# VITA-Group/LightGaussian

Hardware: AMD Instinct MI355X
Metric: views/sec fwd+bwd @1080p (N Gaussians) (higher is better)
Workload: dtype f32; 1 GPU; 3000000 synthetic Gaussians (SURVEY 8d generator, seed 20250103), 1920x1080, SH degree 3, fwdbwd through gaussian_renderer.render, 200-camera orbit; n_gaussians=3000000, width=1920, height=1080, mode=fwdbwd, views=200, exp=hardware, loss=L1 (HIP, lg_loss_forward/backward with LG_FLAG_L1_ONLY), parallelism=camera-shard x1

## Files before the change

### include/lightgaussian.h

```cpp
#ifndef LIGHTGAUSSIAN_H
#define LIGHTGAUSSIAN_H

#include <stddef.h>
#include <stdint.h>

#ifdef __cplusplus
extern "C" {
#endif

#define LG_ABI_VERSION 7

enum {
    LG_OK = 0,
    LG_ERR_INVALID_ARGUMENT = -1,
    LG_ERR_DEVICE = -2,
    LG_ERR_ALLOC = -3,
    LG_ERR_PREFILTERED = -4
};

enum { LG_WEIGHT_ONE = 0, LG_WEIGHT_OPACITY = 1, LG_WEIGHT_ALPHA = 2, LG_WEIGHT_ALPHA_T = 3 };

enum {
    LG_FLAG_DEBUG = 1,
    LG_FLAG_FAST_EXP = 2,
    LG_FLAG_PROFILE = 4,
    LG_FLAG_SKIP_COLOR = 16,
    LG_FLAG_L1_ONLY = 32,
    LG_FLAG_NARROW_KEY = 64,
    LG_FLAG_SORT_ALL_BITS = 128,
    LG_FLAG_K1_LDS = 256,
    LG_FLAG_LONG_SERIAL = 512,
    LG_FLAG_LONG_PARALLEL = 1024,
    LG_FLAG_SAVE_SH_JACOBIAN = 2048,
    LG_FLAG_COUNT_WIDE_BAND = 8192,
    LG_FLAG_RAW_PARAMS = 8
};

typedef struct lg_view {
    int32_t image_height;
    int32_t image_width;
    float tanfovx;
    float tanfovy;
    const float* bg;
    float scale_modifier;
    const float* viewmatrix;
    const float* projmatrix;
    int32_t sh_degree;
    const float* campos;
    int32_t prefiltered;
// ... 116 lines not shown
```

### lightgaussian_amd/_lib.py

```python
import ctypes as C
import os
import subprocess

_HERE = os.path.dirname(os.path.abspath(__file__))
LIB_PATH = os.environ.get("LIGHTGAUSSIAN_HIP_LIB") or os.path.join(_HERE, "liblightgaussian_hip.so")

LG_OK = 0
LG_ERR_INVALID_ARGUMENT = -1
LG_ERR_DEVICE = -2
LG_ERR_ALLOC = -3
LG_ERR_PREFILTERED = -4

WEIGHT_ONE, WEIGHT_OPACITY, WEIGHT_ALPHA, WEIGHT_ALPHA_T = 0, 1, 2, 3
FLAG_DEBUG, FLAG_FAST_EXP, FLAG_PROFILE, FLAG_RAW_PARAMS, FLAG_SKIP_COLOR, FLAG_L1_ONLY = 1, 2, 4, 8, 16, 32
FLAG_NARROW_KEY, FLAG_SORT_ALL_BITS, FLAG_K1_LDS = 64, 128, 256
FLAG_LONG_SERIAL, FLAG_LONG_PARALLEL = 512, 1024
FLAG_SAVE_SH_JACOBIAN = 2048
FLAG_COUNT_WIDE_BAND = 8192
ABI_VERSION = 7

EXPORTS = ["lg_geom_bytes", "lg_img_bytes", "lg_binning_bytes", "lg_backward_scratch_bytes", "lg_forward",
           "lg_forward_count", "lg_backward", "lg_score_from_count", "lg_abi_version", "lg_last_error",
           "lg_profile_read", "lg_profile_reset", "lg_last_stats", "lg_debug_reduce9", "lg_loss_state_bytes",
           "lg_loss_forward", "lg_loss_backward", "lg_prune_scratch_bytes", "lg_prune_epilogue", "lg_knn_scratch_bytes",
           "lg_knn3_mean_dist2", "lg_ordered_sum", "lg_forward_bounded", "lg_select_mask", "lg_compact_scratch_bytes",
           "lg_compact_plan", "lg_compact_rows", "lg_vq_scratch_bytes", "lg_vq_nearest", "lg_debug_sort_temp_bytes",
           "lg_debug_sort_keys", "lg_build_id", "lg_backward_chunked", "lg_debug_activations", "lg_view_status",
           "lg_debug_sort_orphan", "lg_debug_last_contributor", "lg_debug_tile_lists", "lg_geom_visible_offset",
           "lg_sh_grad_from_rgb", "lg_debug_view_meta", "lg_vq_ema_scratch_bytes", "lg_vq_ema_step", "lg_vq_colors"]


class lg_view(C.Structure):
    _fields_ = [("image_height", C.c_int32), ("image_width", C.c_int32), ("tanfovx", C.c_float), ("tanfovy", C.c_float),
# ... 146 lines not shown
```

### lightgaussian_amd/csrc/lg_api.hip

```cpp
#include "lg_host.h"
#include "lg_wave.h"
#include "lg_preprocess.h"
#include "lg_binning.h"
#include "lg_blend.h"
#include "lg_loss.h"
#include "lg_prune.h"
#include "lg_knn.h"
#include "lg_compact.h"
#include "lg_vq.h"
#include "lg_vq_train.h"
#include "lg_vq_color.h"

struct ViewGeom { int W, H, gx, gy, ntiles, ntiles_pad, S, gid_bits; uint32_t gid_mask; };
static ViewGeom view_geom(const lg_view* v, int N)
{
    ViewGeom q;
    q.W = v->image_width; q.H = v->image_height;
    q.gx = (q.W + LG_TILE - 1) / LG_TILE; q.gy = (q.H + LG_TILE - 1) / LG_TILE;
    q.ntiles = (int)((int64_t)q.gx * q.gy);
    q.ntiles_pad = (int)(((int64_t)q.ntiles + LG_TILE_GRID_ALIGN - 1) / LG_TILE_GRID_ALIGN * LG_TILE_GRID_ALIGN);
    q.S = lg_segment_of(v);
    q.gid_bits = lg_gid_bits(N);
    q.gid_mask = lg_gid_mask(q.gid_bits);
    return q;
// ... 44 lines not shown
            if (!g_pin_free.empty()) { p = g_pin_free.back().first; ev = g_pin_free.back().second; g_pin_free.pop_back(); }
        }
        if (!p) {
            if (hipHostMalloc((void**)&p, 64, hipHostMallocDefault) != hipSuccess) { p = nullptr; return; }
            if (hipEventCreateWithFlags(&ev, hipEventDisableTiming) != hipSuccess) { (void)hipHostFree(p); p = nullptr; ev = nullptr; }
        }
    }
    ~PinnedSlot()
    {
        if (p) { std::lock_guard<std::mutex> lk(g_pin_mu); g_pin_free.emplace_back(p, ev); }
    }
    PinnedSlot(const PinnedSlot&) = delete;
    PinnedSlot& operator=(const PinnedSlot&) = delete;
};

#define KCHECK(name)                                                                         \
    do {                                                                                     \
        hipError_t _e = hipGetLastError();                                                   \
        if (_e != hipSuccess) return fail(LG_ERR_DEVICE, name " launch", _e);                \
        if (debug) {                                                                         \
            _e = hipStreamSynchronize(stream);                                               \
            if (_e != hipSuccess) return fail(LG_ERR_DEVICE, name " execution", _e);         \
        }                                                                                    \
    } while (0)

#define LG_STATUS_PENDING 0xFFFFFFFFu

static_assert(LG_W_ALPHA == LG_WEIGHT_ALPHA && LG_W_ALPHA_T == LG_WEIGHT_ALPHA_T, "ForwardPlan::fscore is the kernels' FSCORE");
using PreprocessKernel = decltype(&lg_preprocess<false, false>);
static PreprocessKernel preprocess_kernel(bool raw, bool direct)
{
    static const PreprocessKernel k[2][2] = { { lg_preprocess<false, false>, lg_preprocess<false, true> }, { lg_preprocess<true, false>, lg_preprocess<true, true> } };
    return k[raw][direct];
}
using BlendFwdKernel = decltype(&lg_blend_fwd<false, 0, true, true>);
static BlendFwdKernel blend_fwd_kernel(const ForwardPlan& p)
{
    static const BlendFwdKernel color[2] = { lg_blend_fwd<false, 0, false, true>, lg_blend_fwd<false, 0, true, true> };
    static const BlendFwdKernel count_image[3][2] = { { lg_blend_fwd<true, 0, false, true>, lg_blend_fwd<true, 0, true, true> },
                                                      { lg_blend_fwd<true, LG_W_ALPHA, false, true>, lg_blend_fwd<true, LG_W_ALPHA, true, true> },
                                                      { lg_blend_fwd<true, LG_W_ALPHA_T, false, true>, lg_blend_fwd<true, LG_W_ALPHA_T, true, true> } };
    static const BlendFwdKernel significance[3] = { lg_blend_fwd<true, 0, true, false>, lg_blend_fwd<true, LG_W_ALPHA, true, false>,
                                                    lg_blend_fwd<true, LG_W_ALPHA_T, true, false> };
    const int w = p.fscore == LG_W_ALPHA ? 1 : p.fscore == LG_W_ALPHA_T ? 2 : 0;
    return !p.count ? color[p.exact] : p.color ? count_image[w][p.exact] : significance[w];
}
using BlendBwdKernel = decltype(&lg_blend_bwd<true>);
// ... 3 lines not shown
{
    static const PreprocessBwdKernel k[2][2] = { { lg_preprocess_bwd<false, false>, lg_preprocess_bwd<false, true> },
                                                 { lg_preprocess_bwd<true, false>, lg_preprocess_bwd<true, true> } };
    return k[raw][jac];
}

struct Bounded { void* binning; int64_t capacity; float max_depth; uint32_t* status; uint32_t* host_status; };

struct Forward {
    const lg_view* v; const lg_gaussians* g; const Bounded* bounded; lg_alloc_fn alloc; void* alloc_user; int weight_policy;
    float* out_color; int32_t* out_radii; int32_t* out_count; float* out_score; void** binning_out; int64_t* num_rendered;
    hipStream_t stream; bool debug, prof;
    int N, nblk; ViewGeom q; GeomView geo; ImgView img; BinView bin;
    KeyPlan kp; ForwardPlan plan;
    int64_t cap;
    bool k1_cleared_sort;
    PinnedSlot vslot;
    uint32_t* device_status() const { return bounded ? bounded->status : nullptr; }
    int front_end();
    int binning();
    int blend();
    int score();
    int epilogue();
};

int Forward::front_end()
{
    const bool count = out_count != nullptr;
    if (bounded) {
        if (!bounded->binning || bounded->capacity <= 0 || bounded->capacity >= (1ll << 30) || !(bounded->max_depth > 0.2f))
            return fail(LG_ERR_INVALID_ARGUMENT, "lg_forward_bounded: binning buffer, 0 < max_rendered < 2^30 and max_depth > 0.2 required");
        kp = make_key_plan(q.ntiles, N, __builtin_bit_cast(uint32_t, bounded->max_depth), v->flags);
        cap = bounded->capacity;
        bin = carve_bin(bounded->binning, cap, q.W, q.H, q.S);
        if (N == 0) {
            HIP_TRY(lg_zero_async(geo.counters, 16, stream));
            if (bounded->status) HIP_TRY(lg_zero_async(bounded->status, 16, stream));
            HIP_TRY(lg_zero_async(bin.ranges, (size_t)q.ntiles * 8, stream));
        }
    }
    plan = make_forward_plan(v->flags, count, weight_policy, N, bounded ? cap : 1);
    const bool host_words = bounded && bounded->host_status;
    if (host_words) {
        if (!vslot.p) return fail(LG_ERR_ALLOC, "hipHostMalloc of the status slot failed");
        if (N > 0) { vslot.p[1] = vslot.p[2] = vslot.p[3] = 0u; __atomic_store_n(&vslot.p[0], LG_STATUS_PENDING, __ATOMIC_RELEASE); }
        else memset(vslot.p, 0, 16);
    }
    uint32_t* k1_clear = nullptr;
    uint32_t k1_nclear = 0;
    if (bounded && plan.live) {
        k1_clear = (uint32_t*)bin.sort_temp;
        k1_nclear = (uint32_t)(lg_sort_clear_bytes(lg_sort_layout((size_t)cap), (unsigned)kp.sort_passes()) / 4);
    }
    k1_cleared_sort = k1_clear != nullptr;
    if (N > 0) {
        {
            ProfScope ps(prof, "preprocess", stream);
            const bool direct = !(v->flags & LG_FLAG_K1_LDS), raw = v->flags & LG_FLAG_RAW_PARAMS;
            const size_t k1_dyn = (direct && g->shs && !g->colors_precomp && !plan.k1_skip_color) ? LG_K1_PAD_LDS : 0;
            preprocess_kernel(raw, direct)<<<nblk, LG_PP, k1_dyn, stream>>>(
                N, g->M, v->sh_degree, q.W, q.H, v->tanfovx, v->tanfovy, v->scale_modifier, v->prefiltered, plan.k1_skip_color ? 1 : 0, v->viewmatrix,
                v->projmatrix, v->campos, g->means3D, g->shs, g->shs_rest, g->colors_precomp, g->opacities, g->scales, g->rotations, g->cov3D_precomp, geo,
                out_radii, plan.k1_clears_count ? out_count : nullptr, out_score, k1_clear, k1_nclear, (v->flags & LG_FLAG_SAVE_SH_JACOBIAN) ? 1 : 0);
        }
        KCHECK("lg_preprocess");
        {
            ProfScope ps(prof, "scan", stream);
            lg_scan_blocks<<<(nblk + LG_PART - 1) / LG_PART, LG_PART, 0, stream>>>(nblk, geo.blk_sum, geo.blk_dmax, geo.blk_off, geo.part_sum,
                                                                                  geo.part_dmax, geo.part_prefix, geo.counters + 8,
                                                                                  bounded ? (uint32_t)cap : 0xFFFFFFFFu,
                                                                                  bounded ? kp.depth_bits : 32, geo.counters,
                                                                                  host_words ? vslot.p : device_status());
        }
        KCHECK("lg_scan_blocks");
    }
    if (!bounded) {
        uint32_t h_counters[4] = {0, 0, 0, 0};
        if (N > 0) {
            PinnedSlot slot;
            if (!slot.p) return fail(LG_ERR_ALLOC, "hipHostMalloc of the read-back slot failed");
            HIP_TRY(hipMemcpyAsync(slot.p, geo.counters, 16, hipMemcpyDeviceToHost, stream));
            HIP_TRY(hipStreamSynchronize(stream));
            for (int k = 0; k < 4; k++) h_counters[k] = slot.p[k];
            if (v->prefiltered && h_counters[1]) return fail(LG_ERR_PREFILTERED, "Point is filtered although prefiltered is set. This shouldn't happen!");
            if (h_counters[0] & 1u) return fail(LG_ERR_INVALID_ARGUMENT, "more than 2^32-1 tile instances in one view");
        }
        cap = h_counters[3];
        if (cap >= (1ll << 30)) return fail(LG_ERR_INVALID_ARGUMENT, "more than 2^30-1 tile instances in one view");
        kp = make_key_plan(q.ntiles, N, h_counters[2], v->flags);
        plan = make_forward_plan(v->flags, count, weight_policy, N, cap);
        void* bin_p = alloc(alloc_user, carve_bin(nullptr, cap, q.W, q.H, q.S).total);
        if (!bin_p) return fail(LG_ERR_ALLOC, "binning allocator returned NULL");
        if (binning_out) *binning_out = bin_p;
        bin = carve_bin(bin_p, cap, q.W, q.H, q.S);
        if (num_rendered) *num_rendered = cap;
        if (cap == 0) HIP_TRY(lg_zero_async(bin.ranges, (size_t)q.ntiles * 8, stream));
    }
    g_stats.num_rendered = bounded ? -1 : cap;
    g_stats.num_visible = -1;
    return LG_OK;
}

int Forward::binning()
{
    if (!plan.live) return LG_OK;
    const int sort_begin = kp.sort_begin(), sort_end = kp.sort_end();
    const LgSortLayout SL = lg_sort_layout((size_t)cap);
    if (!k1_cleared_sort) HIP_TRY(lg_zero_async(bin.sort_temp, lg_sort_clear_bytes(SL, (unsigned)kp.sort_passes()), stream));
    uint32_t* hist = (uint32_t*)((char*)bin.sort_temp + SL.hist_off);
    {
        ProfScope ps(prof, "duplicate", stream);
        const int dgrid = std::max(1, std::min((nblk + 4 * LG_DUP_WAVES - 1) / (4 * LG_DUP_WAVES), LG_DUP_GRID));
        lg_duplicate<<<dgrid, LG_DUP_THREADS, 0, stream>>>(N, nblk, q.gx, kp.stored(), kp.store_drop, kp.gid_bits, sort_begin, sort_end, (uint32_t)cap, geo.touched,
                                                          geo.blk_off, geo.part_prefix, geo.counters, geo.offsets, geo.tinfo, bin.keys_in, q.ntiles, bin.ranges, hist,
// ... 109 lines not shown
    if (count && !out_score) return fail(LG_ERR_INVALID_ARGUMENT, "count needs score");
    if (count && (weight_policy < 0 || weight_policy > 3)) return fail(LG_ERR_INVALID_ARGUMENT, "bad weight policy");
    if (count && weight_policy >= LG_WEIGHT_ALPHA && (int64_t)v->image_width * v->image_height > (1ll << 24))
        return fail(LG_ERR_INVALID_ARGUMENT, "ALPHA / ALPHA_T weights: images beyond 2^24 pixels overflow the Q24.40 per-view sums");
    Forward f{};
    f.v = v; f.g = g; f.bounded = bounded; f.alloc = alloc; f.alloc_user = alloc_user; f.weight_policy = weight_policy;
    f.out_color = out_color; f.out_radii = out_radii; f.out_count = out_count; f.out_score = out_score;
    f.binning_out = binning_out; f.num_rendered = num_rendered;
    f.stream = (hipStream_t)stream_p; f.debug = v->flags & LG_FLAG_DEBUG; f.prof = v->flags & LG_FLAG_PROFILE;
    f.N = g->N; f.nblk = (f.N + LG_PP - 1) / LG_PP;
    f.q = view_geom(v, f.N);
    f.geo = carve_geom(geom_p, f.N);
    f.img = carve_img(img_p, f.q.W, f.q.H);
    if (binning_out) *binning_out = nullptr;
    if (num_rendered) *num_rendered = 0;
    if ((rc = f.front_end()) != LG_OK || (rc = f.binning()) != LG_OK || (rc = f.blend()) != LG_OK || (rc = f.score()) != LG_OK) return rc;
    return f.epilogue();
}


extern "C" int lg_forward(const lg_view* view, const lg_gaussians* g, void* geom, void* img, lg_alloc_fn alloc, void* alloc_user,
                          float* out_color, int32_t* out_radii, void** binning_out, int64_t* num_rendered, void* stream)
{
    return forward_impl(view, g, geom, img, alloc, alloc_user, nullptr, LG_WEIGHT_OPACITY, out_color, out_radii, nullptr, nullptr, binning_out,
                        num_rendered, stream);
}

extern "C" int lg_forward_count(const lg_view* view, const lg_gaussians* g, void* geom, void* img, lg_alloc_fn alloc, void* alloc_user,
                                int32_t weight_policy, float* out_color, int32_t* out_radii, int32_t* out_count, float* out_score,
                                void** binning_out, int64_t* num_rendered, void* stream)
{
// ... 652 lines not shown
```

### lightgaussian_amd/csrc/lg_plan.h

```cpp
#pragma once
#include <stdint.h>
#include <algorithm>
#include "../../include/lightgaussian.h"

static inline int bits_for(uint32_t n)
{
    int b = 0;
    while (b < 32 && (1ull << b) < n) b++;
    return b;
}
static inline int lg_gid_bits(int N) { return bits_for((uint32_t)(N > 1 ? N : 2)); }
static inline uint32_t lg_gid_mask(int gid_bits) { return gid_bits >= 32 ? 0xFFFFFFFFu : ((1u << gid_bits) - 1u); }

#define LG_DEPTH_BIAS (124u << 23)
#define LG_NARROW_KEY_BITS 40
struct KeyPlan {
    int tile_bits, gid_bits, depth_bits;
    int store_drop;
    bool two_stage;
    uint32_t gid_mask;
    int stored() const { return depth_bits - store_drop; }
    int tile_shift() const { return gid_bits + stored(); }
    int sort_begin() const { return two_stage ? tile_shift() : gid_bits; }
    int sort_end() const { return tile_shift() + (tile_bits > 0 ? tile_bits : 1); }
// ... 17 lines not shown
enum { LG_SCORE_NONE = 0, LG_SCORE_COUNT = 1, LG_SCORE_COUNT_OPACITY = 2, LG_SCORE_SLOTS = 3 };
struct ForwardPlan {
    bool live;
    bool count;
    bool exact;
    bool color;
    int fscore;
    bool merge;
    bool clear_slots;
    bool k1_skip_color;
    bool k1_clears_count;
    int long_mode;
    int long_chain;
    bool work_list_group;
    int score;
};
static inline ForwardPlan make_forward_plan(uint32_t flags, bool count, int weight_policy, int N, int64_t cap)
{
    const bool fast = flags & LG_FLAG_FAST_EXP;
    const bool want_serial = flags & LG_FLAG_LONG_SERIAL, want_parallel = flags & LG_FLAG_LONG_PARALLEL;
    ForwardPlan p;
    p.live = cap > 0 && N > 0;
    p.count = count;
    p.exact = !fast;
    p.k1_skip_color = flags & LG_FLAG_SKIP_COLOR;
    p.color = !(count && p.exact && p.k1_skip_color);
    p.fscore = (count && (weight_policy == LG_WEIGHT_ALPHA || weight_policy == LG_WEIGHT_ALPHA_T)) ? weight_policy : 0;
    p.merge = p.fscore && !p.color;
    p.clear_slots = p.fscore && !p.merge && p.live;
    p.k1_clears_count = count && !p.fscore;
    p.long_mode = 0;
    p.long_chain = LG_CHAIN_NONE;
    if (p.live && !count && fast) {
        p.long_mode = want_serial ? 0 : want_parallel ? 2 : 1;
        if (p.long_mode) p.long_chain = LG_CHAIN_COLOR;
    } else if (p.live && !p.color && !p.fscore && want_parallel) {
        p.long_mode = 2;
        p.long_chain = LG_CHAIN_COUNT;
    }
    p.work_list_group = p.color || p.long_chain != LG_CHAIN_NONE;
    p.score = !(count && N > 0) ? LG_SCORE_NONE : p.fscore ? LG_SCORE_SLOTS : weight_policy == LG_WEIGHT_OPACITY ? LG_SCORE_COUNT_OPACITY : LG_SCORE_COUNT;
    return p;
}
```

### lightgaussian_amd/csrc/lg_preprocess.h

```cpp
#pragma once

#include "lg_host.h"
#include "lg_wave.h"

#define LG_PP 64
#define LG_ID_BITS 29
#define LG_ID_MASK ((1u << LG_ID_BITS) - 1u)
#define LG_SH_MAXF 48
#ifndef LG_K1_PAD_LDS
#define LG_K1_PAD_LDS 7900
#endif
#ifndef LG_K9_GATHER
#define LG_K9_GATHER 4
#endif
#define LG_COOP_ROWS 48u

__device__ __forceinline__ void stage_sh_rows(const float* __restrict__ shs, int i0, int rows, int rowf, uint64_t need_mask,
                                              float* lds, uint32_t lane)
{
    const float* src = shs + (size_t)i0 * rowf;
    const int nfl = rows * rowf;
    const bool vec_ok = ((reinterpret_cast<uintptr_t>(src) & 15u) == 0);
    if (vec_ok) {
        const int nvec = nfl >> 2;
        for (int q = (int)lane; q < nvec; q += LG_PP) {
            const int f = q << 2;
            if ((rowf & 3) == 0 && !((need_mask >> (f / rowf)) & 1ull)) continue;
            *reinterpret_cast<float4*>(lds + f) = *reinterpret_cast<const float4*>(src + f);
        }
        for (int f = (nvec << 2) + (int)lane; f < nfl; f += LG_PP) lds[f] = src[f];
    } else {
        for (int f = (int)lane; f < nfl; f += LG_PP) lds[f] = src[f];
    }
}

struct __attribute__((packed, aligned(4))) lg_f4u { float x, y, z, w; };
template <int K0>
__device__ __forceinline__ void read_row_direct(const float* __restrict__ row, int nfl, float* sh )
{
#pragma unroll
    for (int q = 0; q < (LG_SH_MAXF - K0 + 3) / 4; q++) {
        float v[4] = {0.0f, 0.0f, 0.0f, 0.0f};
        if (4 * q + 4 <= nfl) {
            const lg_f4u t = reinterpret_cast<const lg_f4u*>(row)[q];
            v[0] = t.x; v[1] = t.y; v[2] = t.z; v[3] = t.w;
        } else {
#pragma unroll
            for (int c = 0; c < 4; c++)
                if (4 * q + c < nfl) v[c] = row[4 * q + c];
        }
#pragma unroll
        for (int c = 0; c < 4; c++)
            if (K0 + 4 * q + c < LG_SH_MAXF) sh[K0 + 4 * q + c] = v[c];
    }
}
__device__ __forceinline__ float lg_sigmoid(float x) { return 1.0f / (1.0f + expf(-x)); }

template <bool RAW, bool DIRECT>
#ifdef LG_K1_WAVES
__global__ void __launch_bounds__(LG_PP) __attribute__((amdgpu_waves_per_eu(LG_K1_WAVES, 8)))
#else
__global__ void __launch_bounds__(LG_PP)
#endif
lg_preprocess(int N, int M, int D, int W, int H, float tanfovx, float tanfovy, float mod, int prefiltered, int skip_color,
              const float* __restrict__ viewmatrix, const float* __restrict__ projmatrix, const float* __restrict__ campos,
              const float* __restrict__ means3D, const float* __restrict__ shs, const float* __restrict__ shs_rest,
              const float* __restrict__ colors_precomp,
              const float* __restrict__ opacities, const float* __restrict__ scales, const float* __restrict__ rotations,
              const float* __restrict__ cov3D_precomp, GeomView g, int32_t* __restrict__ radii, int32_t* __restrict__ zero_count,
              float* __restrict__ zero_score, uint32_t* __restrict__ clear_words, uint32_t n_clear, int save_jac)
{
    __shared__ __attribute__((aligned(16))) float sh_rows[DIRECT ? 4 : LG_PP * LG_SH_MAXF];
    __shared__ float4 st_rec[LG_PP * 3];
    __shared__ __attribute__((aligned(16))) float st_jac[LG_PP * 9];
    static_assert(LG_REC_F4 == 3, "coalesced record store assumes packed 48-byte records");
    const uint32_t lane = threadIdx.x;
    const int i0 = blockIdx.x * LG_PP;
    const int i = i0 + (int)lane;
    for (uint32_t w = blockIdx.x * LG_PP + lane; w < n_clear; w += gridDim.x * LG_PP) clear_words[w] = 0u;
    float vm[16], pm[16], cp[3];
#pragma unroll
    for (int k = 0; k < 16; k++) { vm[k] = viewmatrix[k]; pm[k] = projmatrix[k]; }
    cp[0] = campos[0]; cp[1] = campos[1]; cp[2] = campos[2];
    bool vis = false, violation = false;
    float px = 0, py = 0, pz = 0, op = 0;
    float cov[6] = {0, 0, 0, 0, 0, 0};
    LgSplat sp;
    if (i < N) {
        px = means3D[3 * (size_t)i]; py = means3D[3 * (size_t)i + 1]; pz = means3D[3 * (size_t)i + 2];
        const float vz = vm[2] * px + vm[6] * py + vm[10] * pz + vm[14];
        if (vz > 0.2f) {
            if (cov3D_precomp) {
#pragma unroll
                for (int k = 0; k < 6; k++) cov[k] = cov3D_precomp[6 * (size_t)i + k];
            } else {
                float sc[3] = { scales[3 * (size_t)i], scales[3 * (size_t)i + 1], scales[3 * (size_t)i + 2] };
                const float4 q4 = *reinterpret_cast<const float4*>(rotations + 4 * (size_t)i);
                float q[4] = { q4.x, q4.y, q4.z, q4.w };
                if (RAW) {
                    sc[0] = expf(sc[0]); sc[1] = expf(sc[1]); sc[2] = expf(sc[2]);
                    const float qn = fmaxf(sqrtf((q[0] * q[0] + q[1] * q[1]) + (q[2] * q[2] + q[3] * q[3])), 1e-12f);
                    q[0] /= qn; q[1] /= qn; q[2] /= qn; q[3] /= qn;
                }
                lg_cov3d(sc, mod, q, cov);
            }
            op = RAW ? lg_sigmoid(opacities[i]) : opacities[i];
            vis = lg_project(vm, pm, px, py, pz, cov, op, W, H, tanfovx, tanfovy, sp);
        } else if (prefiltered) {
            violation = true;
        }
        if (zero_count) { zero_count[i] = 0; zero_score[i] = 0.0f; }
    }
    const uint64_t vmask = __ballot(vis);
    const bool split = RAW && shs_rest != nullptr;
    const int rowf = split ? 3 * (M - 1) : 3 * M;
    if (!DIRECT && !skip_color && shs && vmask && rowf > 0) {
        stage_sh_rows(split ? shs_rest : shs, i0, min(LG_PP, N - i0), rowf, vmask, sh_rows, lane);
        __builtin_amdgcn_fence(__ATOMIC_RELEASE, "wavefront");
        __builtin_amdgcn_wave_barrier();
        __builtin_amdgcn_fence(__ATOMIC_ACQUIRE, "wavefront");
    }
    uint32_t touched = 0;
    if (i < N) {
        int radius = 0;
        if (vis) {
            radius = sp.radius;
            touched = (uint32_t)((sp.tx1 - sp.tx0) * (sp.ty1 - sp.ty0));
            float rgb[3] = {0.0f, 0.0f, 0.0f};
            uint32_t cb = 0;
            if (skip_color) {
            } else if (colors_precomp) {
                rgb[0] = colors_precomp[3 * (size_t)i]; rgb[1] = colors_precomp[3 * (size_t)i + 1]; rgb[2] = colors_precomp[3 * (size_t)i + 2];
            } else {
                float sh[LG_SH_MAXF];
                const float* row = DIRECT ? shs + (size_t)i * rowf : sh_rows + lane * rowf;
                const int nact = (D + 1) * (D + 1) * 3;
                if (split && DIRECT) {
                    sh[0] = shs[3 * (size_t)i]; sh[1] = shs[3 * (size_t)i + 1]; sh[2] = shs[3 * (size_t)i + 2];
                    read_row_direct<3>(shs_rest + (size_t)i * rowf, nact - 3, sh);
                } else if (DIRECT) {
                    read_row_direct<0>(row, nact, sh);
                } else if (split) {
                    sh[0] = shs[3 * (size_t)i]; sh[1] = shs[3 * (size_t)i + 1]; sh[2] = shs[3 * (size_t)i + 2];
#pragma unroll
                    for (int k = 3; k < LG_SH_MAXF; k++) sh[k] = (k < nact) ? row[k - 3] : 0.0f;
                } else if ((rowf & 3) == 0) {
#pragma unroll
                    for (int q = 0; q < LG_SH_MAXF / 4; q++) {
                        float4 v4 = make_float4(0, 0, 0, 0);
                        if (q * 4 < nact) v4 = reinterpret_cast<const float4*>(row)[q];
                        sh[4 * q] = v4.x; sh[4 * q + 1] = v4.y; sh[4 * q + 2] = v4.z; sh[4 * q + 3] = v4.w;
                    }
                } else {
#pragma unroll
                    for (int k = 0; k < LG_SH_MAXF; k++) sh[k] = (k < nact) ? row[k] : 0.0f;
                }
                lg_sh_to_rgb(D, sh, px, py, pz, cp, rgb, cb);
                if (save_jac) {
                    float J[9];
                    lg_sh_dir_jacobian(D, sh, px, py, pz, cp, J);
#pragma unroll
                    for (int k = 0; k < 9; k++) st_jac[9 * lane + k] = J[k];
                }
            }
            st_rec[3 * lane + 0] = make_float4(sp.x, sp.y, sp.ha, sp.nb);
            st_rec[3 * lane + 1] = make_float4(sp.hc, op, rgb[0], rgb[1]);
            st_rec[3 * lane + 2] = make_float4(rgb[2], sp.hx, sp.hy, __uint_as_float((uint32_t)i | (cb << LG_ID_BITS)));
            g.tinfo[i] = make_uint4((uint32_t)sp.tx0 | ((uint32_t)sp.ty0 << 16), (uint32_t)sp.tx1 | ((uint32_t)sp.ty1 << 16),
                                    __float_as_uint(sp.depth), 0u);
        }
        radii[i] = radius;
        g.visible[i] = radius > 0 ? (uint8_t)1 : (uint8_t)0;
        g.touched[i] = touched;
    }
    if (vmask) {
        __builtin_amdgcn_fence(__ATOMIC_RELEASE, "wavefront");
        __builtin_amdgcn_wave_barrier();
        __builtin_amdgcn_fence(__ATOMIC_ACQUIRE, "wavefront");
        const int nrec = min(LG_PP, N - i0);
#pragma unroll
        for (int k = 0; k < 3; k++)
            if ((int)(k * LG_PP + lane) < 3 * nrec) g.rec[3 * (size_t)i0 + k * LG_PP + lane] = st_rec[k * LG_PP + lane];
        if (save_jac && shs && !skip_color) {
            float* dstj = g.shjac + 9 * (size_t)i0;
            const int nfl = 9 * nrec, nvec = nfl >> 2;
            for (int q = (int)lane; q < nvec; q += LG_PP) reinterpret_cast<float4*>(dstj)[q] = reinterpret_cast<const float4*>(st_jac)[q];
            for (int f = (nvec << 2) + (int)lane; f < nfl; f += LG_PP) dstj[f] = st_jac[f];
        }
    }
    uint32_t dmax = vis ? __float_as_uint(sp.depth) : 0u;
#pragma unroll
    for (int sh = 32; sh > 0; sh >>= 1) dmax = max(dmax, (uint32_t)__shfl_xor((int)dmax, sh));
    uint32_t tsum = touched;
#pragma unroll
    for (int sh = 32; sh > 0; sh >>= 1) tsum += (uint32_t)__shfl_xor((int)tsum, sh);
    const uint64_t any_violation = __ballot(violation);
    if (lane == 0) {
        g.blk_dmax[blockIdx.x] = dmax | (any_violation ? 0x80000000u : 0u);
        g.blk_sum[blockIdx.x] = tsum;
        if (blockIdx.x == 0) {
            g.counters[8] = 0u;
            g.counters[9] = (save_jac && shs && !skip_color) ? LG_SHJAC_MAGIC : 0u;
        }
    }
}


template <bool RAW, bool JAC>
#ifdef LG_K9_WAVES
__global__ void __launch_bounds__(LG_PP) __attribute__((amdgpu_waves_per_eu(LG_K9_WAVES, 8)))
#else
__global__ void __launch_bounds__(LG_PP)
#endif
lg_preprocess_bwd(int N, int first_blk, int M, int D, int W, int H, float tanfovx, float tanfovy, float mod,
                  const float* __restrict__ viewmatrix, const float* __restrict__ projmatrix, const float* __restrict__ campos,
                  const float* __restrict__ means3D, const float* __restrict__ shs, const float* __restrict__ shs_rest,
                  const float* __restrict__ colors_precomp, const float* __restrict__ opacities,
                  const float* __restrict__ scales, const float* __restrict__ rotations, const float* __restrict__ cov3D_precomp,
// ... 298 lines not shown
```

### lightgaussian_amd/rasterizer.py

```python
import ctypes as C
import threading
from typing import NamedTuple

import torch
import torch.nn as nn

from . import _lib


class GaussianRasterizationSettings(NamedTuple):
    image_height: int
    image_width: int
    tanfovx: float
    tanfovy: float
    bg: torch.Tensor
    scale_modifier: float
    viewmatrix: torch.Tensor
    projmatrix: torch.Tensor
    sh_degree: int
    campos: torch.Tensor
    prefiltered: bool
    debug: bool
    f_count: bool = False


_OPTIONS = {"weight_policy": _lib.WEIGHT_OPACITY, "fast_exp": True, "profile": False, "skip_color_in_count": False,
            "fuse_getters": True, "sync_free": "validated", "max_depth": 100.0, "capacity_margin": 1.25,
            "segment_length": 0, "long_tiles": "auto", "count_long_tiles": "serial",
            "sh_jacobian": True, "narrow_key": False, "sort_all_bits": False, "k1_lds": False, "count_wide_band": False}
_PER_CALL_ONLY = ("pending", "tag", "status_override", "differentiated", "sh_grad_sink", "score_out", "count_sum")
_LONG_TILES = ("serial", "auto", "parallel")
_tls = threading.local()


WEIGHT_POLICIES = {"one": _lib.WEIGHT_ONE, "opacity": _lib.WEIGHT_OPACITY, "alpha": _lib.WEIGHT_ALPHA, "alpha_t": _lib.WEIGHT_ALPHA_T}


def weight_policy_id(value):
    if isinstance(value, str):
        if value.lower() not in WEIGHT_POLICIES:
            raise ValueError(f"weight_policy must be one of {tuple(WEIGHT_POLICIES)} (or a _lib.WEIGHT_* number)")
        return WEIGHT_POLICIES[value.lower()]
    if int(value) not in WEIGHT_POLICIES.values():
# ... 120 lines not shown
        flags = _lib.FLAG_RAW_PARAMS if raw else 0
        if differentiated and opts["sh_jacobian"]:
            flags |= _lib.FLAG_SAVE_SH_JACOBIAN
        if rs.debug:
            flags |= _lib.FLAG_DEBUG
        if opts["fast_exp"] and not exact:
            flags |= _lib.FLAG_FAST_EXP
        if opts["profile"]:
            flags |= _lib.FLAG_PROFILE
        if exact and opts["skip_color_in_count"]:
            flags |= _lib.FLAG_SKIP_COLOR
        if exact:
            flags |= _lib.FLAG_LONG_PARALLEL if opts["count_long_tiles"] == "parallel" else _lib.FLAG_LONG_SERIAL
        else:
            flags |= {"serial": _lib.FLAG_LONG_SERIAL, "auto": 0, "parallel": _lib.FLAG_LONG_PARALLEL}[opts["long_tiles"]]
        if opts["narrow_key"]:
            flags |= _lib.FLAG_NARROW_KEY
        if opts["sort_all_bits"]:
            flags |= _lib.FLAG_SORT_ALL_BITS
        if opts["k1_lds"]:
            flags |= _lib.FLAG_K1_LDS
        if opts["count_wide_band"]:
            flags |= _lib.FLAG_COUNT_WIDE_BAND
        self.view = _lib.lg_view(int(rs.image_height), int(rs.image_width), float(rs.tanfovx), float(rs.tanfovy),
                                 _ptr(self.bg), float(rs.scale_modifier), _ptr(self.vm), _ptr(self.pm),
                                 int(rs.sh_degree), _ptr(self.cp), int(bool(rs.prefiltered)), flags, int(opts["segment_length"]))
        self.g = _lib.lg_gaussians(N, M, _ptr(self.means3D), _ptr(self.sh), _ptr(self.colors), _ptr(self.opac),
                                   _ptr(self.scales), _ptr(self.rots), _ptr(self.cov), _ptr(self.sh_rest))
        self.N, self.M = N, M

# ... 333 lines not shown
```

Measured before the change: 701.6 views/s.

## Split SH colour evaluation into a separate kernel overlapped on a side stream

Moves spherical-harmonic colour evaluation and Jacobian saving out of the preprocess kernel into a new lg_sh_color kernel. When enabled, this kernel runs on a pooled low-priority stream, forked after preprocess and joined before blending, so it can overlap with scan, binning and sorting. The aim is to take the SH evaluation off the critical path and make preprocess lighter. In exchange it adds event and stream overhead, extra partial record writes and a second pass that re-reads means, and colour work now competes with binning for compute units.

```diff
diff --git a/include/lightgaussian.h b/include/lightgaussian.h
--- a/include/lightgaussian.h
+++ b/include/lightgaussian.h
@@ -33,6 +33,7 @@
     LG_FLAG_LONG_PARALLEL = 1024,
     LG_FLAG_SAVE_SH_JACOBIAN = 2048,
     LG_FLAG_COUNT_WIDE_BAND = 8192,
+    LG_FLAG_COLOR_OVERLAP = 16384,
     LG_FLAG_RAW_PARAMS = 8
 };
 
diff --git a/lightgaussian_amd/_lib.py b/lightgaussian_amd/_lib.py
--- a/lightgaussian_amd/_lib.py
+++ b/lightgaussian_amd/_lib.py
@@ -17,6 +17,7 @@
 FLAG_LONG_SERIAL, FLAG_LONG_PARALLEL = 512, 1024
 FLAG_SAVE_SH_JACOBIAN = 2048
 FLAG_COUNT_WIDE_BAND = 8192
+FLAG_COLOR_OVERLAP = 16384
 ABI_VERSION = 7
 
 EXPORTS = ["lg_geom_bytes", "lg_img_bytes", "lg_binning_bytes", "lg_backward_scratch_bytes", "lg_forward",
diff --git a/lightgaussian_amd/csrc/lg_api.hip b/lightgaussian_amd/csrc/lg_api.hip
--- a/lightgaussian_amd/csrc/lg_api.hip
+++ b/lightgaussian_amd/csrc/lg_api.hip
@@ -1,5 +1,8 @@
 #include "lg_host.h"
 #include "lg_wave.h"
+#ifndef LG_COLOR_FORK_AFTER_SCAN
+#define LG_COLOR_FORK_AFTER_SCAN 0
+#endif
 #include "lg_preprocess.h"
 #include "lg_binning.h"
 #include "lg_blend.h"
@@ -82,6 +85,74 @@
     PinnedSlot& operator=(const PinnedSlot&) = delete;
 };
 
+#ifndef LG_COLOR_LANES
+#define LG_COLOR_LANES 8
+#endif
+#ifndef LG_COLOR_LOW_PRIORITY
+#define LG_COLOR_LOW_PRIORITY 1
+#endif
+#ifndef LG_COLOR_WAVES_PER_CU
+#define LG_COLOR_WAVES_PER_CU 8
+#endif
+struct ColorLane { hipStream_t s = nullptr; hipEvent_t forked = nullptr, done = nullptr; int device = -1; int cus = 0; };
+static std::mutex g_lane_mu;
+static std::vector<ColorLane> g_lane_free;
+static int g_lanes_made = 0;
+struct ColorFork {
+    ColorLane lane;
+    hipStream_t caller = nullptr;
+    bool leased = false, launched = false, pending = false;
+    bool lease(hipStream_t caller_stream)
+    {
+        caller = caller_stream;
+        int dev = 0;
+        if (hipGetDevice(&dev) != hipSuccess) return false;
+        {
+            std::lock_guard<std::mutex> lk(g_lane_mu);
+            for (size_t k = 0; k < g_lane_free.size(); k++)
+                if (g_lane_free[k].device == dev) { lane = g_lane_free[k]; g_lane_free.erase(g_lane_free.begin() + (long)k); return leased = true; }
+            if (g_lanes_made >= LG_COLOR_LANES) return false;
+            g_lanes_made++;
+        }
+        ColorLane l;
+        l.device = dev;
+        int lo = 0, hi = 0;
+        bool ok = hipDeviceGetStreamPriorityRange(&lo, &hi) == hipSuccess;
+        ok = ok && hipStreamCreateWithPriority(&l.s, hipStreamNonBlocking, LG_COLOR_LOW_PRIORITY ? lo : 0) == hipSuccess;
+        ok = ok && hipEventCreateWithFlags(&l.forked, hipEventDisableTiming) == hipSuccess;
+        ok = ok && hipEventCreateWithFlags(&l.done, hipEventDisableTiming) == hipSuccess;
+        ok = ok && hipDeviceGetAttribute(&l.cus, hipDeviceAttributeMultiprocessorCount, dev) == hipSuccess && l.cus > 0;
+        if (!ok) {
+            if (l.done) (void)hipEventDestroy(l.done);
+            if (l.forked) (void)hipEventDestroy(l.forked);
+            if (l.s) (void)hipStreamDestroy(l.s);
+            (void)hipGetLastError();
+            std::lock_guard<std::mutex> lk(g_lane_mu);
+            g_lanes_made--;
+            return false;
+        }
+        lane = l;
+        return leased = true;
+    }
+    hipError_t join()
+    {
+        hipError_t e = hipSuccess;
+        if (pending) e = hipStreamWaitEvent(caller, lane.done, 0);
+        else if (launched) e = hipStreamSynchronize(lane.s);
+        if (e != hipSuccess && (pending || launched)) (void)hipStreamSynchronize(lane.s);
+        pending = launched = false;
+        return e;
+    }
+    ~ColorFork()
+    {
+        (void)join();
+        if (leased) { std::lock_guard<std::mutex> lk(g_lane_mu); g_lane_free.push_back(lane); }
+    }
+    ColorFork() = default;
+    ColorFork(const ColorFork&) = delete;
+    ColorFork& operator=(const ColorFork&) = delete;
+};
+
 #define KCHECK(name)                                                                         \
     do {                                                                                     \
         hipError_t _e = hipGetLastError();                                                   \
@@ -95,10 +166,12 @@
 #define LG_STATUS_PENDING 0xFFFFFFFFu
 
 static_assert(LG_W_ALPHA == LG_WEIGHT_ALPHA && LG_W_ALPHA_T == LG_WEIGHT_ALPHA_T, "ForwardPlan::fscore is the kernels' FSCORE");
-using PreprocessKernel = decltype(&lg_preprocess<false, false>);
-static PreprocessKernel preprocess_kernel(bool raw, bool direct)
-{
-    static const PreprocessKernel k[2][2] = { { lg_preprocess<false, false>, lg_preprocess<false, true> }, { lg_preprocess<true, false>, lg_preprocess<true, true> } };
+using PreprocessKernel = decltype(&lg_preprocess<false>);
+static PreprocessKernel preprocess_kernel(bool raw) { return raw ? lg_preprocess<true> : lg_preprocess<false>; }
+using ShColorKernel = decltype(&lg_sh_color<false, false>);
+static ShColorKernel sh_color_kernel(bool raw, bool direct)
+{
+    static const ShColorKernel k[2][2] = { { lg_sh_color<false, false>, lg_sh_color<false, true> }, { lg_sh_color<true, false>, lg_sh_color<true, true> } };
     return k[raw][direct];
 }
 using BlendFwdKernel = decltype(&lg_blend_fwd<false, 0, true, true>);
@@ -132,10 +205,14 @@
     int N, nblk; ViewGeom q; GeomView geo; ImgView img; BinView bin;
     KeyPlan kp; ForwardPlan plan;
     int64_t cap;
+    bool sh_input, capturing;
     bool k1_cleared_sort;
     PinnedSlot vslot;
+    ColorFork fork;
     uint32_t* device_status() const { return bounded ? bounded->status : nullptr; }
     int front_end();
+    int color();
+    int join_color();
     int binning();
     int blend();
     int score();
@@ -145,6 +222,7 @@
 int Forward::front_end()
 {
     const bool count = out_count != nullptr;
+    int rc_color = LG_OK;
     if (bounded) {
         if (!bounded->binning || bounded->capacity <= 0 || bounded->capacity >= (1ll << 30) || !(bounded->max_depth > 0.2f))
             return fail(LG_ERR_INVALID_ARGUMENT, "lg_forward_bounded: binning buffer, 0 < max_rendered < 2^30 and max_depth > 0.2 required");
@@ -157,7 +235,14 @@
             HIP_TRY(lg_zero_async(bin.ranges, (size_t)q.ntiles * 8, stream));
         }
     }
-    plan = make_forward_plan(v->flags, count, weight_policy, N, bounded ? cap : 1);
+    sh_input = g->shs != nullptr && g->colors_precomp == nullptr;
+    capturing = false;
+    if (sh_input && (v->flags & LG_FLAG_COLOR_OVERLAP)) {
+        hipStreamCaptureStatus cs = hipStreamCaptureStatusNone;
+        if (hipStreamIsCapturing(stream, &cs) != hipSuccess) { (void)hipGetLastError(); cs = hipStreamCaptureStatusActive; }
+        capturing = cs != hipStreamCaptureStatusNone;
+    }
+    plan = make_forward_plan(v->flags, count, weight_policy, N, bounded ? cap : 1, sh_input, capturing);
     const bool host_words = bounded && bounded->host_status;
     if (host_words) {
         if (!vslot.p) return fail(LG_ERR_ALLOC, "hipHostMalloc of the status slot failed");
@@ -174,14 +259,16 @@
     if (N > 0) {
         {
             ProfScope ps(prof, "preprocess", stream);
-            const bool direct = !(v->flags & LG_FLAG_K1_LDS), raw = v->flags & LG_FLAG_RAW_PARAMS;
-            const size_t k1_dyn = (direct && g->shs && !g->colors_precomp && !plan.k1_skip_color) ? LG_K1_PAD_LDS : 0;
-            preprocess_kernel(raw, direct)<<<nblk, LG_PP, k1_dyn, stream>>>(
-                N, g->M, v->sh_degree, q.W, q.H, v->tanfovx, v->tanfovy, v->scale_modifier, v->prefiltered, plan.k1_skip_color ? 1 : 0, v->viewmatrix,
-                v->projmatrix, v->campos, g->means3D, g->shs, g->shs_rest, g->colors_precomp, g->opacities, g->scales, g->rotations, g->cov3D_precomp, geo,
-                out_radii, plan.k1_clears_count ? out_count : nullptr, out_score, k1_clear, k1_nclear, (v->flags & LG_FLAG_SAVE_SH_JACOBIAN) ? 1 : 0);
+            const bool jac = plan.color_kernel && (v->flags & LG_FLAG_SAVE_SH_JACOBIAN);
+            preprocess_kernel(v->flags & LG_FLAG_RAW_PARAMS)<<<nblk, LG_PP, 0, stream>>>(
+                N, q.W, q.H, v->tanfovx, v->tanfovy, v->scale_modifier, v->prefiltered, plan.color_kernel ? 1 : 0, v->viewmatrix, v->projmatrix,
+                g->means3D, g->colors_precomp, g->opacities, g->scales, g->rotations, g->cov3D_precomp, geo, out_radii,
+                plan.k1_clears_count ? out_count : nullptr, out_score, k1_clear, k1_nclear, jac ? 1 : 0);
         }
         KCHECK("lg_preprocess");
+#if !LG_COLOR_FORK_AFTER_SCAN
+        if ((rc_color = color()) != LG_OK) return rc_color;
+#endif
         {
             ProfScope ps(prof, "scan", stream);
             lg_scan_blocks<<<(nblk + LG_PART - 1) / LG_PART, LG_PART, 0, stream>>>(nblk, geo.blk_sum, geo.blk_dmax, geo.blk_off, geo.part_sum,
@@ -191,6 +278,9 @@
                                                                                   host_words ? vslot.p : device_status());
         }
         KCHECK("lg_scan_blocks");
+#if LG_COLOR_FORK_AFTER_SCAN
+        if ((rc_color = color()) != LG_OK) return rc_color;
+#endif
     }
     if (!bounded) {
         uint32_t h_counters[4] = {0, 0, 0, 0};
@@ -206,7 +296,7 @@
         cap = h_counters[3];
         if (cap >= (1ll << 30)) return fail(LG_ERR_INVALID_ARGUMENT, "more than 2^30-1 tile instances in one view");
         kp = make_key_plan(q.ntiles, N, h_counters[2], v->flags);
-        plan = make_forward_plan(v->flags, count, weight_policy, N, cap);
+        plan = make_forward_plan(v->flags, count, weight_policy, N, cap, sh_input, capturing);
         void* bin_p = alloc(alloc_user, carve_bin(nullptr, cap, q.W, q.H, q.S).total);
         if (!bin_p) return fail(LG_ERR_ALLOC, "binning allocator returned NULL");
         if (binning_out) *binning_out = bin_p;
@@ -216,6 +306,45 @@
     }
     g_stats.num_rendered = bounded ? -1 : cap;
     g_stats.num_visible = -1;
+    return LG_OK;
+}
+
+int Forward::color()
+{
+    if (!plan.color_kernel) return LG_OK;
+    const bool direct = !(v->flags & LG_FLAG_K1_LDS), raw = v->flags & LG_FLAG_RAW_PARAMS;
+    const int save_jac = (v->flags & LG_FLAG_SAVE_SH_JACOBIAN) ? 1 : 0;
+    const bool forked = plan.color_fork && fork.lease(stream);
+    if (!forked) {
+        ProfScope ps(prof, "preprocess_color", stream);
+        sh_color_kernel(raw, direct)<<<nblk, LG_PP, direct ? LG_COLOR_PAD_LDS : 0, stream>>>(N, nblk, g->M, v->sh_degree, v->campos, g->means3D, g->shs,
+                                                                                         g->shs_rest, geo, save_jac);
+        KCHECK("lg_sh_color");
+        return LG_OK;
+    }
+    HIP_TRY(hipEventRecord(fork.lane.forked, stream));
+    HIP_TRY(hipStreamWaitEvent(fork.lane.s, fork.lane.forked, 0));
+    const int grid = LG_COLOR_WAVES_PER_CU > 0 ? std::min(nblk, fork.lane.cus * LG_COLOR_WAVES_PER_CU) : nblk;
+    const size_t dyn = (LG_COLOR_WAVES_PER_CU > 0 || !direct) ? 0 : LG_COLOR_PAD_LDS;
+    sh_color_kernel(raw, direct)<<<grid, LG_PP, dyn, fork.lane.s>>>(N, nblk, g->M, v->sh_degree, v->campos, g->means3D, g->shs, g->shs_rest, geo, save_jac);
+    {
+        const hipError_t e = hipGetLastError();
+        if (e != hipSuccess) return fail(LG_ERR_DEVICE, "lg_sh_color launch", e);
+    }
+    fork.launched = true;
+    HIP_TRY(hipEventRecord(fork.lane.done, fork.lane.s));
+    fork.pending = true;
+    if (debug) {
+        const hipError_t e = hipStreamSynchronize(fork.lane.s);
+        if (e != hipSuccess) return fail(LG_ERR_DEVICE, "lg_sh_color execution", e);
+    }
+    return LG_OK;
+}
+
+int Forward::join_color()
+{
+    const hipError_t e = fork.join();
+    if (e != hipSuccess) return fail(LG_ERR_DEVICE, "join of the colour stream", e);
     return LG_OK;
 }
 
@@ -355,7 +484,7 @@
     f.img = carve_img(img_p, f.q.W, f.q.H);
     if (binning_out) *binning_out = nullptr;
     if (num_rendered) *num_rendered = 0;
-    if ((rc = f.front_end()) != LG_OK || (rc = f.binning()) != LG_OK || (rc = f.blend()) != LG_OK || (rc = f.score()) != LG_OK) return rc;
+    if ((rc = f.front_end()) != LG_OK || (rc = f.binning()) != LG_OK || (rc = f.join_color()) != LG_OK || (rc = f.blend()) != LG_OK || (rc = f.score()) != LG_OK) return rc;
     return f.epilogue();
 }
 
diff --git a/lightgaussian_amd/csrc/lg_plan.h b/lightgaussian_amd/csrc/lg_plan.h
--- a/lightgaussian_amd/csrc/lg_plan.h
+++ b/lightgaussian_amd/csrc/lg_plan.h
@@ -55,8 +55,11 @@
     int long_chain;
     bool work_list_group;
     int score;
+    bool color_kernel;
+    bool color_fork;
 };
-static inline ForwardPlan make_forward_plan(uint32_t flags, bool count, int weight_policy, int N, int64_t cap)
+static inline ForwardPlan make_forward_plan(uint32_t flags, bool count, int weight_policy, int N, int64_t cap, bool sh_input = false,
+                                            bool capturing = false)
 {
     const bool fast = flags & LG_FLAG_FAST_EXP;
     const bool want_serial = flags & LG_FLAG_LONG_SERIAL, want_parallel = flags & LG_FLAG_LONG_PARALLEL;
@@ -80,6 +83,8 @@
         p.long_chain = LG_CHAIN_COUNT;
     }
     p.work_list_group = p.color || p.long_chain != LG_CHAIN_NONE;
+    p.color_kernel = p.color && !p.k1_skip_color && sh_input && N > 0;
+    p.color_fork = p.color_kernel && (flags & LG_FLAG_COLOR_OVERLAP) && !(flags & LG_FLAG_PROFILE) && !capturing;
     p.score = !(count && N > 0) ? LG_SCORE_NONE : p.fscore ? LG_SCORE_SLOTS : weight_policy == LG_WEIGHT_OPACITY ? LG_SCORE_COUNT_OPACITY : LG_SCORE_COUNT;
     return p;
 }
diff --git a/lightgaussian_amd/csrc/lg_preprocess.h b/lightgaussian_amd/csrc/lg_preprocess.h
--- a/lightgaussian_amd/csrc/lg_preprocess.h
+++ b/lightgaussian_amd/csrc/lg_preprocess.h
@@ -7,9 +7,6 @@
 #define LG_ID_BITS 29
 #define LG_ID_MASK ((1u << LG_ID_BITS) - 1u)
 #define LG_SH_MAXF 48
-#ifndef LG_K1_PAD_LDS
-#define LG_K1_PAD_LDS 7900
-#endif
 #ifndef LG_K9_GATHER
 #define LG_K9_GATHER 4
 #endif
@@ -35,6 +32,7 @@
 }
 
 struct __attribute__((packed, aligned(4))) lg_f4u { float x, y, z, w; };
+struct __attribute__((packed, aligned(4))) lg_f2u { float x, y; };
 template <int K0>
 __device__ __forceinline__ void read_row_direct(const float* __restrict__ row, int nfl, float* sh )
 {
@@ -56,32 +54,28 @@
 }
 __device__ __forceinline__ float lg_sigmoid(float x) { return 1.0f / (1.0f + expf(-x)); }
 
-template <bool RAW, bool DIRECT>
+template <bool RAW>
 #ifdef LG_K1_WAVES
 __global__ void __launch_bounds__(LG_PP) __attribute__((amdgpu_waves_per_eu(LG_K1_WAVES, 8)))
 #else
 __global__ void __launch_bounds__(LG_PP)
 #endif
-lg_preprocess(int N, int M, int D, int W, int H, float tanfovx, float tanfovy, float mod, int prefiltered, int skip_color,
-              const float* __restrict__ viewmatrix, const float* __restrict__ projmatrix, const float* __restrict__ campos,
-              const float* __restrict__ means3D, const float* __restrict__ shs, const float* __restrict__ shs_rest,
-              const float* __restrict__ colors_precomp,
+lg_preprocess(int N, int W, int H, float tanfovx, float tanfovy, float mod, int prefiltered, int sep_color,
+              const float* __restrict__ viewmatrix, const float* __restrict__ projmatrix,
+              const float* __restrict__ means3D, const float* __restrict__ colors_precomp,
               const float* __restrict__ opacities, const float* __restrict__ scales, const float* __restrict__ rotations,
               const float* __restrict__ cov3D_precomp, GeomView g, int32_t* __restrict__ radii, int32_t* __restrict__ zero_count,
-              float* __restrict__ zero_score, uint32_t* __restrict__ clear_words, uint32_t n_clear, int save_jac)
+              float* __restrict__ zero_score, uint32_t* __restrict__ clear_words, uint32_t n_clear, int jac_marker)
 {
-    __shared__ __attribute__((aligned(16))) float sh_rows[DIRECT ? 4 : LG_PP * LG_SH_MAXF];
     __shared__ float4 st_rec[LG_PP * 3];
-    __shared__ __attribute__((aligned(16))) float st_jac[LG_PP * 9];
     static_assert(LG_REC_F4 == 3, "coalesced record store assumes packed 48-byte records");
     const uint32_t lane = threadIdx.x;
     const int i0 = blockIdx.x * LG_PP;
     const int i = i0 + (int)lane;
     for (uint32_t w = blockIdx.x * LG_PP + lane; w < n_clear; w += gridDim.x * LG_PP) clear_words[w] = 0u;
-    float vm[16], pm[16], cp[3];
+    float vm[16], pm[16];
 #pragma unroll
     for (int k = 0; k < 16; k++) { vm[k] = viewmatrix[k]; pm[k] = projmatrix[k]; }
-    cp[0] = campos[0]; cp[1] = campos[1]; cp[2] = campos[2];
     bool vis = false, violation = false;
     float px = 0, py = 0, pz = 0, op = 0;
     float cov[6] = {0, 0, 0, 0, 0, 0};
@@ -112,14 +106,6 @@
         if (zero_count) { zero_count[i] = 0; zero_score[i] = 0.0f; }
     }
     const uint64_t vmask = __ballot(vis);
-    const bool split = RAW && shs_rest != nullptr;
-    const int rowf = split ? 3 * (M - 1) : 3 * M;
-    if (!DIRECT && !skip_color && shs && vmask && rowf > 0) {
-        stage_sh_rows(split ? shs_rest : shs, i0, min(LG_PP, N - i0), rowf, vmask, sh_rows, lane);
-        __builtin_amdgcn_fence(__ATOMIC_RELEASE, "wavefront");
-        __builtin_amdgcn_wave_barrier();
-        __builtin_amdgcn_fence(__ATOMIC_ACQUIRE, "wavefront");
-    }
     uint32_t touched = 0;
     if (i < N) {
         int radius = 0;
@@ -127,45 +113,12 @@
             radius = sp.radius;
             touched = (uint32_t)((sp.tx1 - sp.tx0) * (sp.ty1 - sp.ty0));
             float rgb[3] = {0.0f, 0.0f, 0.0f};
-            uint32_t cb = 0;
-            if (skip_color) {
-            } else if (colors_precomp) {
+            if (colors_precomp) {
                 rgb[0] = colors_precomp[3 * (size_t)i]; rgb[1] = colors_precomp[3 * (size_t)i + 1]; rgb[2] = colors_precomp[3 * (size_t)i + 2];
-            } else {
-                float sh[LG_SH_MAXF];
-                const float* row = DIRECT ? shs + (size_t)i * rowf : sh_rows + lane * rowf;
-                const int nact = (D + 1) * (D + 1) * 3;
-                if (split && DIRECT) {
-                    sh[0] = shs[3 * (size_t)i]; sh[1] = shs[3 * (size_t)i + 1]; sh[2] = shs[3 * (size_t)i + 2];
-                    read_row_direct<3>(shs_rest + (size_t)i * rowf, nact - 3, sh);
-                } else if (DIRECT) {
-                    read_row_direct<0>(row, nact, sh);
-                } else if (split) {
-                    sh[0] = shs[3 * (size_t)i]; sh[1] = shs[3 * (size_t)i + 1]; sh[2] = shs[3 * (size_t)i + 2];
-#pragma unroll
-                    for (int k = 3; k < LG_SH_MAXF; k++) sh[k] = (k < nact) ? row[k - 3] : 0.0f;
-                } else if ((rowf & 3) == 0) {
-#pragma unroll
-                    for (int q = 0; q < LG_SH_MAXF / 4; q++) {
-                        float4 v4 = make_float4(0, 0, 0, 0);
-                        if (q * 4 < nact) v4 = reinterpret_cast<const float4*>(row)[q];
-                        sh[4 * q] = v4.x; sh[4 * q + 1] = v4.y; sh[4 * q + 2] = v4.z; sh[4 * q + 3] = v4.w;
-                    }
-                } else {
-#pragma unroll
-                    for (int k = 0; k < LG_SH_MAXF; k++) sh[k] = (k < nact) ? row[k] : 0.0f;
-                }
-                lg_sh_to_rgb(D, sh, px, py, pz, cp, rgb, cb);
-                if (save_jac) {
-                    float J[9];
-                    lg_sh_dir_jacobian(D, sh, px, py, pz, cp, J);
-#pragma unroll
-                    for (int k = 0; k < 9; k++) st_jac[9 * lane + k] = J[k];
-                }
             }
             st_rec[3 * lane + 0] = make_float4(sp.x, sp.y, sp.ha, sp.nb);
             st_rec[3 * lane + 1] = make_float4(sp.hc, op, rgb[0], rgb[1]);
-            st_rec[3 * lane + 2] = make_float4(rgb[2], sp.hx, sp.hy, __uint_as_float((uint32_t)i | (cb << LG_ID_BITS)));
+            st_rec[3 * lane + 2] = make_float4(rgb[2], sp.hx, sp.hy, __uint_as_float((uint32_t)i));
             g.tinfo[i] = make_uint4((uint32_t)sp.tx0 | ((uint32_t)sp.ty0 << 16), (uint32_t)sp.tx1 | ((uint32_t)sp.ty1 << 16),
                                     __float_as_uint(sp.depth), 0u);
         }
@@ -179,13 +132,15 @@
         __builtin_amdgcn_fence(__ATOMIC_ACQUIRE, "wavefront");
         const int nrec = min(LG_PP, N - i0);
 #pragma unroll
-        for (int k = 0; k < 3; k++)
-            if ((int)(k * LG_PP + lane) < 3 * nrec) g.rec[3 * (size_t)i0 + k * LG_PP + lane] = st_rec[k * LG_PP + lane];
-        if (save_jac && shs && !skip_color) {
-            float* dstj = g.shjac + 9 * (size_t)i0;
-            const int nfl = 9 * nrec, nvec = nfl >> 2;
-            for (int q = (int)lane; q < nvec; q += LG_PP) reinterpret_cast<float4*>(dstj)[q] = reinterpret_cast<const float4*>(st_jac)[q];
-            for (int f = (nvec << 2) + (int)lane; f < nfl; f += LG_PP) dstj[f] = st_jac[f];
+        for (int k = 0; k < 3; k++) {
+            const int e = k * LG_PP + (int)lane;
+            if (e < 3 * nrec) {
+                const float4 v = st_rec[e];
+                float* dst = reinterpret_cast<float*>(g.rec + 3 * (size_t)i0 + e);
+                if (!sep_color || e % 3 == 0) *reinterpret_cast<float4*>(dst) = v;
+                else if (e % 3 == 1) *reinterpret_cast<float2*>(dst) = make_float2(v.x, v.y);
+                else { lg_f2u h; h.x = v.y; h.y = v.z; *reinterpret_cast<lg_f2u*>(dst + 1) = h; }
+            }
         }
     }
     uint32_t dmax = vis ? __float_as_uint(sp.depth) : 0u;
@@ -200,8 +155,90 @@
         g.blk_sum[blockIdx.x] = tsum;
         if (blockIdx.x == 0) {
             g.counters[8] = 0u;
-            g.counters[9] = (save_jac && shs && !skip_color) ? LG_SHJAC_MAGIC : 0u;
-        }
+            g.counters[9] = jac_marker ? LG_SHJAC_MAGIC : 0u;
+        }
+    }
+}
+
+#ifndef LG_COLOR_PAD_LDS
+#define LG_COLOR_PAD_LDS 11000
+#endif
+template <bool RAW, bool DIRECT>
+__global__ void __launch_bounds__(LG_PP)
+lg_sh_color(int N, int nblk, int M, int D, const float* __restrict__ campos, const float* __restrict__ means3D,
+            const float* __restrict__ shs, const float* __restrict__ shs_rest, GeomView g, int save_jac)
+{
+    __shared__ __attribute__((aligned(16))) float sh_rows[DIRECT ? 4 : LG_PP * LG_SH_MAXF];
+    __shared__ __attribute__((aligned(16))) float st_jac[LG_PP * 9];
+    const uint32_t lane = threadIdx.x;
+    float cp[3];
+    cp[0] = campos[0]; cp[1] = campos[1]; cp[2] = campos[2];
+    const bool split = RAW && shs_rest != nullptr;
+    const int rowf = split ? 3 * (M - 1) : 3 * M;
+    for (int blk = (int)blockIdx.x; blk < nblk; blk += (int)gridDim.x) {
+        const int i0 = blk * LG_PP;
+        const int i = i0 + (int)lane;
+        const bool vis = i < N && g.visible[i] != 0;
+        const uint64_t vmask = __ballot(vis);
+        if (!vmask) continue;
+        if (!DIRECT && rowf > 0) {
+            stage_sh_rows(split ? shs_rest : shs, i0, min(LG_PP, N - i0), rowf, vmask, sh_rows, lane);
+            __builtin_amdgcn_fence(__ATOMIC_RELEASE, "wavefront");
+            __builtin_amdgcn_wave_barrier();
+            __builtin_amdgcn_fence(__ATOMIC_ACQUIRE, "wavefront");
+        }
+        if (vis) {
+            const float px = means3D[3 * (size_t)i], py = means3D[3 * (size_t)i + 1], pz = means3D[3 * (size_t)i + 2];
+            float rgb[3] = {0.0f, 0.0f, 0.0f};
+            uint32_t cb = 0;
+            float sh[LG_SH_MAXF];
+            const float* row = DIRECT ? shs + (size_t)i * rowf : sh_rows + lane * rowf;
+            const int nact = (D + 1) * (D + 1) * 3;
+            if (split && DIRECT) {
+                sh[0] = shs[3 * (size_t)i]; sh[1] = shs[3 * (size_t)i + 1]; sh[2] = shs[3 * (size_t)i + 2];
+                read_row_direct<3>(shs_rest + (size_t)i * rowf, nact - 3, sh);
+            } else if (DIRECT) {
+                read_row_direct<0>(row, nact, sh);
+            } else if (split) {
+                sh[0] = shs[3 * (size_t)i]; sh[1] = shs[3 * (size_t)i + 1]; sh[2] = shs[3 * (size_t)i + 2];
+#pragma unroll
+                for (int k = 3; k < LG_SH_MAXF; k++) sh[k] = (k < nact) ? row[k - 3] : 0.0f;
+            } else if ((rowf & 3) == 0) {
+#pragma unroll
+                for (int q = 0; q < LG_SH_MAXF / 4; q++) {
+                    float4 v4 = make_float4(0, 0, 0, 0);
+                    if (q * 4 < nact) v4 = reinterpret_cast<const float4*>(row)[q];
+                    sh[4 * q] = v4.x; sh[4 * q + 1] = v4.y; sh[4 * q + 2] = v4.z; sh[4 * q + 3] = v4.w;
+                }
+            } else {
+#pragma unroll
+                for (int k = 0; k < LG_SH_MAXF; k++) sh[k] = (k < nact) ? row[k] : 0.0f;
+            }
+            lg_sh_to_rgb(D, sh, px, py, pz, cp, rgb, cb);
+            if (save_jac) {
+                float J[9];
+                lg_sh_dir_jacobian(D, sh, px, py, pz, cp, J);
+#pragma unroll
+                for (int k = 0; k < 9; k++) st_jac[9 * lane + k] = J[k];
+            }
+            float* rw = reinterpret_cast<float*>(g.rec + LG_REC_F4 * (size_t)i);
+            *reinterpret_cast<float2*>(rw + 6) = make_float2(rgb[0], rgb[1]);
+            rw[8] = rgb[2];
+            rw[11] = __uint_as_float((uint32_t)i | (cb << LG_ID_BITS));
+        }
+        if (save_jac) {
+            __builtin_amdgcn_fence(__ATOMIC_RELEASE, "wavefront");
+            __builtin_amdgcn_wave_barrier();
+            __builtin_amdgcn_fence(__ATOMIC_ACQUIRE, "wavefront");
+            const int nrec = min(LG_PP, N - i0);
+            float* dstj = g.shjac + 9 * (size_t)i0;
+            const int nfl = 9 * nrec, nvec = nfl >> 2;
+            for (int q = (int)lane; q < nvec; q += LG_PP) reinterpret_cast<float4*>(dstj)[q] = reinterpret_cast<const float4*>(st_jac)[q];
+            for (int f = (nvec << 2) + (int)lane; f < nfl; f += LG_PP) dstj[f] = st_jac[f];
+        }
+        __builtin_amdgcn_fence(__ATOMIC_RELEASE, "wavefront");
+        __builtin_amdgcn_wave_barrier();
+        __builtin_amdgcn_fence(__ATOMIC_ACQUIRE, "wavefront");
     }
 }
 
diff --git a/lightgaussian_amd/rasterizer.py b/lightgaussian_amd/rasterizer.py
--- a/lightgaussian_amd/rasterizer.py
+++ b/lightgaussian_amd/rasterizer.py
@@ -1,4 +1,5 @@
 import ctypes as C
+import os
 import threading
 from typing import NamedTuple
 
@@ -27,6 +28,7 @@
 _OPTIONS = {"weight_policy": _lib.WEIGHT_OPACITY, "fast_exp": True, "profile": False, "skip_color_in_count": False,
             "fuse_getters": True, "sync_free": "validated", "max_depth": 100.0, "capacity_margin": 1.25,
             "segment_length": 0, "long_tiles": "auto", "count_long_tiles": "serial",
+            "color_overlap": os.environ.get("LG_COLOR_OVERLAP", "1") != "0",
             "sh_jacobian": True, "narrow_key": False, "sort_all_bits": False, "k1_lds": False, "count_wide_band": False}
 _PER_CALL_ONLY = ("pending", "tag", "status_override", "differentiated", "sh_grad_sink", "score_out", "count_sum")
 _LONG_TILES = ("serial", "auto", "parallel")
@@ -177,6 +179,8 @@
             flags |= _lib.FLAG_LONG_PARALLEL if opts["count_long_tiles"] == "parallel" else _lib.FLAG_LONG_SERIAL
         else:
             flags |= {"serial": _lib.FLAG_LONG_SERIAL, "auto": 0, "parallel": _lib.FLAG_LONG_PARALLEL}[opts["long_tiles"]]
+        if opts["color_overlap"]:
+            flags |= _lib.FLAG_COLOR_OVERLAP
         if opts["narrow_key"]:
             flags |= _lib.FLAG_NARROW_KEY
         if opts["sort_all_bits"]:
```

Result: slower. 652.0 views/s (-7.1%).
